# ooowedyn/InkLayer

Hardware: AMD Instinct MI355X
Metric: sketches/sec end-to-end (GroundingDINO+SAM) at 1024x1024 (higher is better)
Workload: dtype f16 (MFMA, f32 accumulate; f32 residual/norm/softmax; split-f16 = fp32-grade operands for patch-embed, neck, mask decoder); 1 GPU; full GroundingDINO Swin-T + SAM ViT-H pipeline, batch=8 per GPU, 1024x1024 synthetic sketches, 16 boxes/sketch, random-init weights; global_batch=8, parallelism=image-parallel x1

## Files before the change

### include/inklayer_hip.h

```cpp
#ifndef INKLAYER_HIP_H
#define INKLAYER_HIP_H

#include <stdint.h>

#ifdef __cplusplus
extern "C" {
#endif

#define INK_ABI_VERSION 10
int ink_abi_version(void);

typedef struct InkGemm {
  const void* A;
  const void* W;
  const float* bias;
  const float* col_scale;
  const float* residual;
  const int32_t* row_map;
  void* C;
  int32_t M, N, K;
  int32_t lda, ldw, ldr, ldc;
  int32_t act;
  int32_t c_f16;
} InkGemm;
// ... 106 lines not shown

int ink_groupnorm_nhwc(const float* x, int32_t B, int32_t T, int32_t C, int32_t G, const float* gamma,
                       const float* beta, float eps, float* stats_ws, float* out,
                       int64_t out_batch_stride, void* stream);

int ink_gather_rows(const float* x, int64_t ldx, int64_t x_batch_rows, const int32_t* idx,
                    int64_t idx_batch_stride, int32_t rows_per_batch, int32_t B, int32_t C,
                    void* out_f16, float* out_f32, void* stream);

int ink_attn_fewkeys(const void* Q, int64_t ldq, const void* K, int64_t ldk, const void* V, int64_t ldv,
                     int32_t B, int32_t n_q, int32_t n_k, int32_t n_heads, int32_t head_dim, float scale,
                     const uint8_t* blocked, const int32_t* q_batch_rows, const float* q_add, int32_t io_f32, void* O,
                     int64_t ldo, void* stream);

int ink_attn_midkeys(const void* Q, int64_t ldq, const void* K, int64_t ldk, const void* V, int64_t ldv, int32_t B,
                     int32_t n_q, int32_t n_k, int32_t n_heads, int32_t head_dim, float scale, const uint8_t* blocked,
                     void* O, int64_t ldo, void* stream);

int ink_biattn_wide_workspace(int32_t B, int32_t S, int32_t T, int64_t* out_floats);
int ink_biattn_wide(const void* QV_f16, const void* KL_f16, int32_t B, int32_t S, int32_t T, int32_t E, float scale,
                    float* ws, void* out_v_f16, void* out_l_f16, void* stream);

int ink_attn_fewq(const void* Q, int64_t ldq, const void* K, int64_t ldk, const void* V, int64_t ldv,
                  int32_t n_batch, int32_t n_q, int32_t n_k, int32_t n_heads, int32_t head_dim, float scale,
                  const int32_t* q_batch_rows, const int32_t* kv_batch_rows, const float* k_add, void* O, int64_t ldo,
                  void* stream);

int ink_biattn_colstats(const float* scores, int32_t B, int32_t S, int32_t HT, float* part_ws, float* stats, void* stream);

int ink_fusion_fold_workspace(int32_t B, int32_t S, int64_t* out_floats);
int ink_fusion_fold(float* v_f32, int32_t B, int32_t S, const float* lnv_g, const float* lnv_b, float eps,
                    const float* text_k_f32, const float* text_vl_f32, int64_t ld_text, int32_t T, const void* Wq_f16,
                    const float* bq, const void* Wvv_f16, const float* bvv, const void* Wo_f16, const float* bo,
                    const float* gamma_v, float scale, float* ws, void* out_l_f16, const float* pos, void* out16_pos,
                    void* out16, void* stream);

int ink_sam_upscale_pack(const void* ws_f16, void* blob_f16, void* stream);
int ink_sam_upscale_tail(const float* u0, int64_t ld_tok, int32_t n, int32_t g, const float* ln_g, const float* ln_b, float eps,
                         const void* blob_f16, const float* b3, const float* hyper, int32_t n_masks, float* low,
                         void* stream);

int ink_proj256_ln_pack(const void* ws_f16, void* blob_f16, void* stream);
int ink_proj256_ln(const float* a_f32, const void* blob_f16, const float* bias, const float* res_f32,
                   const int32_t* res_batch_rows, int32_t rows_per_batch, const float* ln_g, const float* ln_b, float eps,
                   int64_t rows, float* out_f32, void* out_split_f16, void* stream);

int ink_ffn256_pack_bytes(int32_t hid, int32_t with_pre, int64_t* out_bytes);
int ink_ffn256_pack(const void* w1_f16, const float* b1, const void* w2_f16, int32_t hid, const void* wpre_f16, void* blob,
                    void* stream);
int ink_ffn256_fused(const void* x_f16, int64_t ldx, const float* res_f32, const void* blob, const float* b2,
                     const float* ln_g, const float* ln_b, float eps, int32_t M, int32_t hid, const float* pre_bias,
                     const float* pre_ln_g, const float* pre_ln_b, float* out_f32, void* stream);

int ink_topk_rowmax(const float* logits, int32_t B, int32_t S, int32_t T, int32_t K, int32_t* out_idx,
                    float* out_val, void* cand_ws, void* stream);

int ink_sine_embed4(const float* ref, const float* dim_t, int32_t N, void* out_f16, void* stream);

int ink_box_refine(const float* delta, int64_t ldd, const float* ref, int32_t N, int32_t ref_is_logit,
                   float* out, void* stream);

int ink_mask_cleanup_workspace_ints(int32_t n, int32_t H, int32_t W, int32_t k, int64_t* out_ints);
int ink_mask_cleanup(const void* masks_u8, int32_t n, int32_t H, int32_t W, int32_t k, int32_t area_threshold,
                     double aspect_threshold, void* tmp_a_u8, void* tmp_b_u8, int32_t* workspace, void* out_u8,
                     void* stream);

int ink_mask_sketch_iou_counts(const void* masks_u8, const void* sketch_rgb_u8, int32_t n, int32_t H, int32_t W,
                               void* bits_ws_u64, int32_t* counts, void* stream);

int ink_sam_amg_stats(const float* low, int32_t n, const int32_t* index, int32_t m, const int32_t* m_dev, int32_t S,
                      int32_t L, int32_t in_h, int32_t in_w, int32_t crop_h, int32_t crop_w, double thr, double offset,
                      int32_t x0, int32_t y0, int32_t orig_h, int32_t orig_w, int32_t* table, void* planes_u64,
                      float* out_logits, void* stream);

int ink_mask_rle_counts(const void* planes_u64, const int32_t* select, int32_t k, int32_t H, int32_t W,
                        int32_t* n_counts, void* stream);
int ink_mask_rle_write(const void* planes_u64, const int32_t* select, int32_t k, int32_t H, int32_t W,
                       const int32_t* offsets, int32_t* counts, void* stream);

int ink_mask_small_regions_workspace_ints(int32_t k, int32_t H, int32_t W, int64_t* out_ints);
int ink_mask_small_regions(const void* planes_u64, int32_t k, int32_t H, int32_t W, int32_t min_area, int32_t holes,
                           void* tmp_planes_u64, int32_t* workspace, void* out_planes_u64, int32_t* changed, void* stream);

int ink_box_nms(const float* boxes, const float* scores, int32_t n, float iou_threshold, void* workspace_u64,
                int32_t* keep, int32_t* n_keep, void* stream);

int ink_refine_sketch_planes(const void* rgb_u8, int32_t H, int32_t W, void* planes4_u64, int32_t* max_ws, void* stream);

int ink_bitplane_pack(const void* img_u8, int32_t n, int32_t H, int32_t W, int32_t thresh, void* planes_u64, void* stream);

int ink_refine_depth_samples(const void* mask_planes, int32_t n, const float* depth, const int32_t* pts_yx, int32_t P,
                             int32_t H, int32_t W, float* vals, void* inside_u8, void* stream);

int ink_refine_pair_tables(const void* mask_planes, const void* sketch_planes4, int32_t n, int32_t H, int32_t W,
                           const int32_t* rect, void* dil_ws_planes, int32_t* pair, int32_t* per_mask,
                           int32_t* sketch_area, void* stream);

int ink_refine_composite(const void* mask_planes, const int32_t* order, int32_t n_ranks, int32_t H, int32_t W,
                         void* label_u8, int32_t* hist256, void* stream);

int ink_refine_relabel_clean(const void* label_u8, const void* map256_u8, int32_t H, int32_t W, void* out_label_u8,
                             void* stream);

int ink_refine_grow_workspace(int32_t H, int32_t W, int64_t* plane_words, int64_t* cc_ints);
int ink_refine_grow(const void* label_u8, const void* sketch_planes4, int32_t H, int32_t W, void* planes_ws,
                    int32_t* cc_ws, int32_t* flags256, void* out_label_u8, int32_t* bbox256x4, int32_t* unl_yx,
// ... 104 lines not shown
```

### inklayer_amd/_lib.py

```python
from __future__ import annotations

import ctypes as C
import os
from pathlib import Path

_LIB_PATH = Path(__file__).resolve().parent / "lib" / "libinklayer_hip.so"
_lib = None

c_void_p, c_int, c_i64, c_float = C.c_void_p, C.c_int32, C.c_int64, C.c_float


class InkGemm(C.Structure):
    _fields_ = [
        ("A", c_void_p), ("W", c_void_p), ("bias", c_void_p), ("col_scale", c_void_p),
        ("residual", c_void_p), ("row_map", c_void_p), ("C", c_void_p),
        ("M", c_int), ("N", c_int), ("K", c_int),
        ("lda", c_int), ("ldw", c_int), ("ldr", c_int), ("ldc", c_int),
        ("act", c_int), ("c_f16", c_int),
    ]


class InkAttn(C.Structure):
    _fields_ = [
        ("Q", c_void_p), ("K", c_void_p), ("V", c_void_p), ("O", c_void_p),
# ... 20 lines not shown
    "ink_flash_attn": [C.POINTER(InkAttn), c_void_p],
    "ink_swin_attn": [c_void_p, c_void_p, c_void_p, c_i64, c_i64, c_i64, c_void_p, c_i64, c_int, c_int, c_int, c_float,
                      c_void_p, c_void_p, c_int, c_void_p],
    "ink_sam_patchify": [c_void_p, c_int, c_int, c_int, c_int, C.POINTER(c_float), C.POINTER(c_float),
                         c_int, c_int, c_void_p, c_void_p],
    "ink_im2col3x3_f16": [c_void_p, c_int, c_int, c_int, c_int, c_int, c_int, c_void_p, c_void_p],
    "ink_resize_u8": [c_void_p, c_int, c_int, c_int, c_void_p, c_int, c_int, c_void_p, c_void_p, c_int,
                      c_void_p, c_void_p, c_int, c_void_p, c_void_p],
    "ink_sam_pe_encode": [c_void_p, c_void_p, c_int, c_int, c_void_p, c_int, c_void_p, c_void_p],
    "ink_sam_mask_logits": [c_void_p, c_void_p, c_int, c_int, c_int, c_void_p, c_void_p],
    "ink_sam_prompt_tokens": [c_void_p, c_void_p, c_int, c_int, c_void_p, c_void_p, c_int, c_void_p, c_void_p,
                              c_void_p, c_float, c_int, c_void_p, c_void_p],
    "ink_sam_mask_embed": [c_void_p, c_void_p, c_void_p, c_void_p, c_int, c_float, c_int, c_int, c_void_p, c_void_p,
                           c_void_p],
    "ink_sam_postprocess": [c_void_p, c_int, c_int, c_int, c_int, c_int, c_int, c_int, c_float,
                            c_void_p, c_void_p, c_void_p],
    "ink_sam_amg_stats": [c_void_p, c_int, c_void_p, c_int, c_void_p, c_int, c_int, c_int, c_int, c_int, c_int, C.c_double,
                          C.c_double, c_int, c_int, c_int, c_int, c_void_p, c_void_p, c_void_p, c_void_p],
    "ink_mask_rle_counts": [c_void_p, c_void_p, c_int, c_int, c_int, c_void_p, c_void_p],
    "ink_mask_rle_write": [c_void_p, c_void_p, c_int, c_int, c_int, c_void_p, c_void_p, c_void_p],
    "ink_mask_small_regions_workspace_ints": [c_int, c_int, c_int, C.POINTER(c_i64)],
    "ink_mask_small_regions": [c_void_p, c_int, c_int, c_int, c_int, c_int, c_void_p, c_void_p, c_void_p, c_void_p,
                               c_void_p],
    "ink_box_nms": [c_void_p, c_void_p, c_int, c_float, c_void_p, c_void_p, c_void_p, c_void_p],
    "ink_ms_deform_attn_forward": [c_void_p, C.POINTER(c_i64), C.POINTER(c_i64), c_void_p, c_void_p, c_int,
                                   c_int, c_int, c_int, c_int, c_int, c_int, c_int, c_void_p, c_void_p],
    "ink_ms_deform_attn_forward_dev": [c_void_p, c_void_p, c_void_p, c_void_p, c_void_p, c_int, c_int, c_int, c_int,
                                       c_int, c_int, c_int, c_int, c_int, c_void_p, c_void_p],
    "ink_ms_deform_attn_backward_dev": [c_void_p, c_void_p, c_void_p, c_void_p, c_void_p, c_void_p, c_int, c_int, c_int,
                                        c_int, c_int, c_int, c_int, c_int, c_int, c_void_p, c_void_p, c_void_p,
                                        c_void_p],
    "ink_msda_fused": [c_void_p, c_void_p, c_i64, c_void_p, c_int, c_i64, c_i64, C.POINTER(c_int), c_int,
                       c_int, c_int, c_void_p, c_void_p],
    "ink_swin_patchify": [c_void_p, c_int, c_int, C.POINTER(c_float), C.POINTER(c_float), c_void_p, c_void_p],
    "ink_layernorm_merge4": [c_void_p, c_i64, c_void_p, c_void_p, c_float, c_void_p, c_int, c_int, c_void_p,
                             c_void_p],
    "ink_groupnorm_nhwc": [c_void_p, c_int, c_int, c_int, c_int, c_void_p, c_void_p, c_float, c_void_p,
                           c_void_p, c_i64, c_void_p],
    "ink_gather_rows": [c_void_p, c_i64, c_i64, c_void_p, c_i64, c_int, c_int, c_int, c_void_p, c_void_p,
                        c_void_p],
    "ink_biattn_colstats": [c_void_p, c_int, c_int, c_int, c_void_p, c_void_p, c_void_p],
    "ink_fusion_fold_workspace": [c_int, c_int, C.POINTER(c_i64)],
    "ink_relpos_bias64_f16": [c_void_p, c_i64, c_void_p, c_void_p, c_int, c_int, c_int, c_float, c_void_p, c_void_p, c_void_p],
    "ink_proj256_ln_pack": [c_void_p, c_void_p, c_void_p],
    "ink_proj256_ln": [c_void_p, c_void_p, c_void_p, c_void_p, c_void_p, c_int, c_void_p, c_void_p, c_float, c_i64, c_void_p,
                       c_void_p, c_void_p],
    "ink_sam_upscale_pack": [c_void_p, c_void_p, c_void_p],
    "ink_sam_upscale_tail": [c_void_p, c_i64, c_int, c_int, c_void_p, c_void_p, c_float, c_void_p, c_void_p, c_void_p,
                             c_int, c_void_p, c_void_p],
    "ink_ffn256_pack_bytes": [c_int, c_int, C.POINTER(c_i64)],
    "ink_ffn256_pack": [c_void_p, c_void_p, c_void_p, c_int, c_void_p, c_void_p, c_void_p],
    "ink_ffn256_fused": [c_void_p, c_i64, c_void_p, c_void_p, c_void_p, c_void_p, c_void_p, c_float, c_int, c_int,
                         c_void_p, c_void_p, c_void_p, c_void_p, c_void_p],
    "ink_fusion_fold": [c_void_p, c_int, c_int, c_void_p, c_void_p, c_float, c_void_p, c_void_p, c_i64, c_int, c_void_p,
                        c_void_p, c_void_p, c_void_p, c_void_p, c_void_p, c_void_p, c_float, c_void_p, c_void_p, c_void_p,
                        c_void_p, c_void_p, c_void_p],
    "ink_attn_fewkeys": [c_void_p, c_i64, c_void_p, c_i64, c_void_p, c_i64, c_int, c_int, c_int, c_int, c_int,
                         c_float, c_void_p, c_void_p, c_void_p, c_int, c_void_p, c_i64, c_void_p],
    "ink_attn_midkeys": [c_void_p, c_i64, c_void_p, c_i64, c_void_p, c_i64, c_int, c_int, c_int, c_int, c_int,
                         c_float, c_void_p, c_void_p, c_i64, c_void_p],
    "ink_biattn_wide_workspace": [c_int, c_int, c_int, C.POINTER(c_i64)],
    "ink_biattn_wide": [c_void_p, c_void_p, c_int, c_int, c_int, c_int, c_float, c_void_p, c_void_p, c_void_p,
                        c_void_p],
    "ink_attn_fewq": [c_void_p, c_i64, c_void_p, c_i64, c_void_p, c_i64, c_int, c_int, c_int, c_int, c_int,
                      c_float, c_void_p, c_void_p, c_void_p, c_void_p, c_i64, c_void_p],
    "ink_topk_rowmax": [c_void_p, c_int, c_int, c_int, c_int, c_void_p, c_void_p, c_void_p, c_void_p],
    "ink_sine_embed4": [c_void_p, c_void_p, c_int, c_void_p, c_void_p],
    "ink_box_refine": [c_void_p, c_i64, c_void_p, c_int, c_int, c_void_p, c_void_p],
    "ink_mask_cleanup_workspace_ints": [c_int, c_int, c_int, c_int, C.POINTER(c_i64)],
    "ink_mask_cleanup": [c_void_p, c_int, c_int, c_int, c_int, c_int, C.c_double, c_void_p, c_void_p, c_void_p,
                         c_void_p, c_void_p],
    "ink_mask_sketch_iou_counts": [c_void_p, c_void_p, c_int, c_int, c_int, c_void_p, c_void_p, c_void_p],
    "ink_refine_sketch_planes": [c_void_p, c_int, c_int, c_void_p, c_void_p, c_void_p],
    "ink_bitplane_pack": [c_void_p, c_int, c_int, c_int, c_int, c_void_p, c_void_p],
    "ink_refine_depth_samples": [c_void_p, c_int, c_void_p, c_void_p, c_int, c_int, c_int, c_void_p, c_void_p, c_void_p],
    "ink_refine_pair_tables": [c_void_p, c_void_p, c_int, c_int, c_int, c_void_p, c_void_p, c_void_p, c_void_p,
                               c_void_p, c_void_p],
    "ink_refine_composite": [c_void_p, c_void_p, c_int, c_int, c_int, c_void_p, c_void_p, c_void_p],
    "ink_refine_relabel_clean": [c_void_p, c_void_p, c_int, c_int, c_void_p, c_void_p],
    "ink_refine_grow_workspace": [c_int, c_int, C.POINTER(c_i64), C.POINTER(c_i64)],
    "ink_refine_grow": [c_void_p, c_void_p, c_int, c_int, c_void_p, c_void_p, c_void_p, c_void_p, c_void_p, c_void_p,
                        c_int, c_void_p, c_void_p],
    "ink_refine_query_dists": [c_void_p, c_void_p, c_void_p, c_int, c_int, c_int, c_void_p, c_void_p],
    "ink_refine_finalize": [c_void_p, c_void_p, c_int, c_void_p, c_int, c_int, c_void_p, c_void_p, c_void_p, c_void_p],
    "ink_host_sparse_sample": [c_void_p, c_int, c_int, c_void_p, c_int, c_void_p],
    "ink_host_assign_unlabeled": [c_void_p, c_int, c_void_p, c_int, c_void_p, c_void_p, c_void_p, c_int, c_void_p],
    "ink_depth_patchify": [c_void_p, c_int, c_int, c_int, c_int, c_int, c_int, C.POINTER(C.c_double), C.POINTER(C.c_double),
                           c_int, c_void_p, c_void_p],
    "ink_resize_bilinear_ac_nhwc": [c_void_p, c_int, c_int, c_int, c_int, c_int, c_int, c_void_p, c_void_p, c_void_p],
    "ink_conv3x3_f16": [c_void_p, c_int, c_int, c_int, c_int, c_void_p, c_int, c_void_p, c_int, c_int, c_int, c_void_p,
                        c_void_p, c_int, c_void_p],
    "ink_layers_otsu_planes": [c_void_p, c_int, c_int, c_int, c_int, c_void_p, c_void_p, c_void_p, c_void_p],
    "ink_layers_dilate": [c_void_p, c_int, c_int, c_int, c_int, c_int, c_void_p, c_void_p, c_void_p],
    "ink_layers_border_band": [c_void_p, c_int, c_int, c_int, c_int, c_void_p, c_void_p],
    "ink_layers_components_workspace_ints": [c_int, c_int, c_int, C.POINTER(c_i64)],
    "ink_layers_components": [c_void_p, c_int, c_int, c_int, c_int, c_void_p, c_void_p, c_void_p, c_void_p],
    "ink_layers_chamfer_workspace_ints": [c_int, c_int, c_int, C.POINTER(c_i64)],
    "ink_layers_chamfer": [c_void_p, c_void_p, c_int, c_int, c_int, c_int, c_int, c_void_p, c_void_p, c_void_p, c_void_p,
                           c_void_p, c_void_p],
    "ink_layers_mask_tables": [c_void_p, c_int, c_int, c_int, c_void_p, c_void_p, c_void_p],
    "ink_layers_assemble": [c_void_p, c_void_p, c_void_p, c_void_p, c_void_p, c_int, c_int, c_int, c_void_p, c_void_p,
                            c_void_p, c_void_p],
    "ink_layers_composite": [c_void_p, c_void_p, c_int, c_int, c_void_p, c_void_p],
    "ink_layers_gray": [c_void_p, c_int, c_int, c_int, c_void_p, c_void_p],
    "ink_layers_rgba": [c_void_p, c_void_p, c_int, c_int, c_int, c_void_p, c_void_p],
    "ink_inp_contrast": [c_void_p, c_int, c_int, c_float, c_void_p, c_void_p, c_void_p],
# ... 53 lines not shown
```

### inklayer_amd/build.py

```python
from __future__ import annotations

import os
import subprocess
import sys
from concurrent.futures import ThreadPoolExecutor
from pathlib import Path

ROOT = Path(__file__).resolve().parent
CSRC = ROOT / "csrc"
LIBDIR = ROOT / "lib"
OBJDIR = LIBDIR / "obj"
LIB = LIBDIR / "libinklayer_hip.so"
HIPCC = os.environ.get("HIPCC", "/opt/rocm/bin/hipcc")
FLAGS = ["--offload-arch=gfx950", "-O3", "-std=c++17", "-fPIC", "-ffp-contract=off",
         "-mllvm", "-amdgpu-mfma-vgpr-form",

         "-Wall", "-Wno-unused-function", "-Wno-unused-variable"]


def _newest_header() -> float:
    hs = list(CSRC.glob("*.h")) + list((ROOT.parent / "include").glob("*.h"))
    return max(h.stat().st_mtime for h in hs)


NO_SPILL = {"ffn_fused.hip", "proj_ln.hip", "amg.hip", "layers.hip", "inpaint_ops.hip", "visualize.hip", "evaluate.hip",
            "gemm.hip", "attention_swin.hip", "biattn_wide.hip"}


def _check_no_spill(src: Path, remarks: str) -> None:
    name = None
    for line in remarks.splitlines():
        if "Function Name:" in line:
            name = line.split("Function Name:")[1].split("[")[0].strip()
        elif "ScratchSize [bytes/lane]:" in line:
            n = int(line.split("ScratchSize [bytes/lane]:")[1].split("[")[0])
            if n != 0:
                raise RuntimeError(f"{src.name}: kernel {name} spills ({n} bytes of scratch per lane) - the kernels of "
                                   f"this file must stay in registers (see NO_SPILL); reduce register pressure")


def _compile(src: Path, force: bool, hdr_time: float) -> Path:
    obj = OBJDIR / (src.stem + ".o")
    if (not force and obj.exists() and obj.stat().st_mtime > src.stat().st_mtime
            and obj.stat().st_mtime > hdr_time):
        return obj
    guard = src.name in NO_SPILL
    cmd = [HIPCC, *FLAGS, *(["-Rpass-analysis=kernel-resource-usage", "-fno-caret-diagnostics"] if guard else []), "-c", str(src), "-o", str(obj)]
    r = subprocess.run(cmd, capture_output=True, text=True)
    if r.returncode != 0:
        raise RuntimeError(f"hipcc failed for {src.name}:\n{r.stdout}\n{r.stderr}")
    err = r.stderr
    if guard:
        try:
            _check_no_spill(src, err)
        except RuntimeError:
            obj.unlink(missing_ok=True)
            raise
        err = "\n".join(l for l in err.splitlines()
                        if "kernel-resource-usage" not in l and not l.startswith("In file included from"))
    if err.strip():
        sys.stderr.write(err)
    return obj


def build(force: bool = False, verbose: bool = True) -> Path:
    OBJDIR.mkdir(parents=True, exist_ok=True)
    srcs = sorted(CSRC.glob("*.hip"))
    if not srcs:
        raise RuntimeError("no HIP sources found")
    hdr_time = _newest_header()
    with ThreadPoolExecutor(max_workers=min(8, len(srcs))) as ex:
        objs = list(ex.map(lambda s: _compile(s, force, hdr_time), srcs))
    if (force or not LIB.exists()
            or any(o.stat().st_mtime > LIB.stat().st_mtime for o in objs)):
        cmd = [HIPCC, "--offload-arch=gfx950", "-shared", "-fPIC", "-o", str(LIB),
               *map(str, objs)]
        r = subprocess.run(cmd, capture_output=True, text=True)
        if r.returncode != 0:
            raise RuntimeError(f"link failed:\n{r.stdout}\n{r.stderr}")
# ... 8 lines not shown
```

### inklayer_amd/gdino.py

```python
from __future__ import annotations

import math
from dataclasses import dataclass, replace
from typing import Dict, List, Optional, Sequence, Tuple

import numpy as np
import torch

from . import ops
from ._lru import LRU

F16, F32, I32 = torch.float16, torch.float32, torch.int32


@dataclass
class GDinoConfig:
    embed_dim: int = 96
    depths: Tuple[int, ...] = (2, 2, 6, 2)
    num_heads: Tuple[int, ...] = (3, 6, 12, 24)
    window_size: int = 7
    out_indices: Tuple[int, ...] = (1, 2, 3)
    hidden_dim: int = 256
    nheads: int = 8
    enc_layers: int = 6
# ... 287 lines not shown
        return {(k[7:] if k.startswith("module.") else k): v for k, v in sd.items()}
    return sd


class GDinoEngine:
    fuse_ffn = True
    fuse_ffn_pre = True
    fold_fusion = True

    def __init__(self, state_dict: Dict[str, torch.Tensor], cfg: Optional[GDinoConfig] = None,
                 device: str | torch.device = "cuda", encoded_text: Optional[torch.Tensor] = None,
                 token_ids: Sequence[int] = DEFAULT_TOKEN_IDS):
        cfg = cfg or GDinoConfig()
        self.cfg, self.dev = cfg, torch.device(device)
        assert self.dev.type == "cuda", "the InkLayer detector runs on MI355X only"
        check_config(cfg)
        sd, dev = clean_state_dict(state_dict), self.dev
        self.w: Dict[str, torch.Tensor] = {}
        w = self.w

        def h(name, shape=None):
            t = sd[name].detach().to(torch.float32)
            return (t.reshape(shape) if shape is not None else t).to(dev, F16).contiguous()

        def f(name):
            return ops.own_f32(sd[name], dev)

        def lin(dst, src):
            w[dst + ".w"], w[dst + ".b"] = h(src + ".weight"), f(src + ".bias")

        def ln(dst, src):
            w[dst + ".w"], w[dst + ".b"] = f(src + ".weight"), f(src + ".bias")

        def cat_lin(dst, srcs):
            w[dst + ".w"] = torch.cat([h(s + ".weight") for s in srcs]).contiguous()
            w[dst + ".b"] = torch.cat([f(s + ".bias") for s in srcs]).contiguous()

        bb = "backbone.0."
        pw = sd[bb + "patch_embed.proj.weight"].detach().to(torch.float32).cpu().reshape(cfg.embed_dim, 48)
        w["pe.w"] = torch.cat([pw, torch.zeros(cfg.embed_dim, 16)], 1).to(dev, F16).contiguous()
        w["pe.b"] = f(bb + "patch_embed.proj.bias")
        ln("pe.norm", bb + "patch_embed.norm")
        ws = cfg.window_size
        scale = HEAD_DIM ** -0.5
        for i, (dep, nh) in enumerate(zip(cfg.depths, cfg.num_heads)):
            for b in range(dep):
                p, d = f"{bb}layers.{i}.blocks.{b}.", f"s{i}b{b}"
                ln(d + ".norm1", p + "norm1")
                ln(d + ".norm2", p + "norm2")
                lin(d + ".qkv", p + "attn.qkv")
                lin(d + ".proj", p + "attn.proj")
                lin(d + ".fc1", p + "mlp.fc1")
                lin(d + ".fc2", p + "mlp.fc2")
                tab = sd[p + "attn.relative_position_bias_table"].detach().to(torch.float32).cpu()
                if ws == 7:
                    w[d + ".bias"] = swin_dense_bias(tab, ws, nh, scale).to(dev).contiguous()
                else:
                    w[d + ".table"] = swin_bias_table(tab, ws, nh).to(dev).contiguous()
            if i < len(cfg.depths) - 1:
                ln(f"s{i}.merge.norm", f"{bb}layers.{i}.downsample.norm")
                w[f"s{i}.merge.w"] = h(f"{bb}layers.{i}.downsample.reduction.weight")
            if i in cfg.out_indices:
                ln(f"s{i}.outnorm", f"{bb}norm{i}")
        for l in range(cfg.num_feature_levels):
            cw = sd[f"input_proj.{l}.0.weight"].detach().to(torch.float32)
            if cw.shape[-1] == 1:
                w[f"ip{l}.w"] = cw.reshape(cw.shape[0], cw.shape[1]).to(dev, F16).contiguous()
            else:
                w[f"ip{l}.w"] = cw.permute(0, 2, 3, 1).reshape(cw.shape[0], -1).to(dev, F16).contiguous()
            w[f"ip{l}.b"] = f(f"input_proj.{l}.0.bias")
            ln(f"ip{l}.gn", f"input_proj.{l}.1")
        t = "transformer."
        self.level_embed_cpu = sd[t + "level_embed"].detach().to(torch.float32).cpu()

        def msda(dst, src):
            cat_lin(dst + ".proj", [src + "sampling_offsets", src + "attention_weights"])
            lin(dst + ".value", src + "value_proj")
            lin(dst + ".out", src + "output_proj")

        def mha(dst, src):
            W, b = sd[src + "in_proj_weight"].detach().to(torch.float32), sd[src + "in_proj_bias"].detach().to(torch.float32)
            D = W.shape[1]
            w[dst + ".qk.w"], w[dst + ".qk.b"] = W[:2 * D].to(dev, F16).contiguous(), b[:2 * D].to(dev).contiguous()
            w[dst + ".q.w"], w[dst + ".q.b"] = W[:D].to(dev, F16).contiguous(), b[:D].to(dev).contiguous()
            w[dst + ".kv.w"], w[dst + ".kv.b"] = W[D:].to(dev, F16).contiguous(), b[D:].to(dev).contiguous()
            w[dst + ".v.w"], w[dst + ".v.b"] = W[2 * D:].to(dev, F16).contiguous(), b[2 * D:].to(dev).contiguous()
            lin(dst + ".out", src + "out_proj")

        for i in range(cfg.enc_layers):
            p, d = f"{t}encoder.layers.{i}.", f"e{i}"
            msda(d + ".msda", p + "self_attn.")
            ln(d + ".norm1", p + "norm1"); lin(d + ".lin1", p + "linear1"); lin(d + ".lin2", p + "linear2"); ln(d + ".norm2", p + "norm2")
            if w[d + ".lin1.w"].shape[1] == 256 and w[d + ".lin1.w"].shape[0] % 64 == 0 and w[d + ".lin1.w"].shape[0] <= 2048:
                w[d + ".ffn.blob"] = ops.ffn256_pack(w[d + ".lin1.w"], w[d + ".lin1.b"], w[d + ".lin2.w"])
                w[d + ".ffn.blob_pre"] = ops.ffn256_pack(w[d + ".lin1.w"], w[d + ".lin1.b"], w[d + ".lin2.w"],
                                                         w[d + ".msda.out.w"])
            p = f"{t}encoder.text_layers.{i}."
            mha(d + ".txt", p + "self_attn.")
            lin(d + ".txt.lin1", p + "linear1"); lin(d + ".txt.lin2", p + "linear2")
            ln(d + ".txt.norm1", p + "norm1"); ln(d + ".txt.norm2", p + "norm2")
            p = f"{t}encoder.fusion_layers.{i}."
            ln(d + ".fu.lnv", p + "layer_norm_v"); ln(d + ".fu.lnl", p + "layer_norm_l")
            cat_lin(d + ".fu.qv", [p + "attn.v_proj", p + "attn.values_v_proj"])
            cat_lin(d + ".fu.kl", [p + "attn.l_proj", p + "attn.values_l_proj"])
            lin(d + ".fu.outv", p + "attn.out_v_proj"); lin(d + ".fu.outl", p + "attn.out_l_proj")
            w[d + ".fu.gv"], w[d + ".fu.gl"] = f(p + "gamma_v"), f(p + "gamma_l")
# ... 41 lines not shown
        self._graphs.clear()
        self._seen.clear()
        self.T = T
        self.token_ids = tuple(int(t) for t in token_ids)
        self._text_attn = ops.attn_fewkeys if T <= 16 else ops.attn_midkeys
        self.text0 = encoded_text.detach().to(self.dev, F32).contiguous()
        self._captions.put(self.token_ids, encoded_text.detach().to("cpu", F32))
        self.Tc, self.logit_bias = -(-T // 4) * 4, None
        if self.Tc != T:
            self.logit_bias = torch.zeros(self.Tc, dtype=F32)
            self.logit_bias[T:] = float("-inf")
            self.logit_bias = self.logit_bias.to(self.dev)
        sm, pid = text_masks_and_position_ids(token_ids)
        self.text_blocked = (~sm).to(torch.uint8).to(self.dev).contiguous()
        dim_t = torch.arange(256, dtype=torch.float32)
        dim_t = 10000.0 ** (2 * torch.div(dim_t, 2, rounding_mode="floor") / 256)
        self.pos_text = _interleaved_sincos(pid.float()[:, None] * (2 * math.pi) / dim_t).to(self.dev).contiguous()

    caption_cache_size = 8
    tokenizer = None

    def set_caption(self, token_ids: Sequence[int], sd: Optional[Dict[str, torch.Tensor]] = None,
                    encoded_text: Optional[torch.Tensor] = None) -> None:
        ids = tuple(int(t) for t in token_ids)[:self.cfg.max_text_len]
        if sd is not None:
            sd = clean_state_dict(sd)
            self.text_weights = {k: v for k, v in sd.items() if k.startswith(("bert.", "feat_map."))}
            self._captions.clear()
        if encoded_text is None:
            encoded_text = self._captions.get(ids)
        if encoded_text is None:
            if not self.text_weights:
                raise ValueError("set_caption needs encoded_text [T, 256] or a state dict with the checkpoint's bert.* "
                                 "and feat_map.* tensors")
            from .text_branch import encode_caption_from_checkpoint
            encoded_text = encode_caption_from_checkpoint(self.text_weights, ids)
        self.set_text(encoded_text[:len(ids)], ids)

    def predict(self, images_u8: Sequence[torch.Tensor], box_threshold: float, text_threshold: float,
                remove_combined: bool = False):
        logits, boxes = self.forward(images_u8)
        both = torch.cat([logits, boxes], dim=-1).cpu()
        T, res = self.T, []
        for b in range(both.shape[0]):
            prob = both[b, :, :T].contiguous().sigmoid()
            keep = prob.max(dim=1)[0] > box_threshold
            kept = prob[keep]
            phrases = phrases_from_probs(kept, self.token_ids, text_threshold, remove_combined, self.tokenizer)
            res.append((both[b, keep, T:], kept.max(dim=1)[0] if len(kept) else kept.new_zeros(0), phrases))
        return res

    graph_max_batch = 1
    graph_cache_size = 4
    plan_cache_size = 8

    def _forward_graphed(self, images_u8: Sequence[torch.Tensor], h: int, w_: int):
        B = len(images_u8)
        key = (h, w_, B)
        g = self._graphs.get(key)
        if g is None:
            self._seen[key] = self._seen.get(key, 0) + 1
            if len(self._seen) > 4096:
                self._seen.clear()
            if self._seen[key] < 2:
                return self._forward_eager(images_u8)
            static_in = [torch.empty_like(im) for im in images_u8]
            for dst, src in zip(static_in, images_u8):
                dst.copy_(src)
            side = torch.cuda.Stream(device=self.dev)
            side.wait_stream(torch.cuda.current_stream(self.dev))
            with torch.cuda.stream(side):
                for _ in range(2):
                    self._forward_eager(static_in)
            torch.cuda.current_stream(self.dev).wait_stream(side)
            graph = torch.cuda.CUDAGraph()
            with torch.cuda.graph(graph):
                out = self._forward_eager(static_in)
            g = (graph, static_in, out, self.plan(h, w_, B))
            self._graphs.put(key, g)
        graph, static_in, out = g[:3]
        for dst, src in zip(static_in, images_u8):
            dst.copy_(src)
        graph.replay()
        return out[0].clone(), out[1].clone()

    def plan(self, h: int, w: int, B: int) -> _Plan:
        return self._plans.get_or_make((h, w, B), lambda: _Plan(self, h, w, B))

    def _mlp3(self, prefix: str, x16: torch.Tensor) -> torch.Tensor:
        w = self.w
        a = ops.gemm(x16, w[prefix + "0.w"], w[prefix + "0.b"], act="relu", out_dtype=F16)
        a = ops.gemm(a, w[prefix + "1.w"], w[prefix + "1.b"], act="relu", out_dtype=F16)
        return ops.gemm(a, w[prefix + "2.w"], w[prefix + "2.b"])

    def _swin_block(self, x: torch.Tensor, i: int, b: int, pl: _Plan) -> None:
        cfg, w = self.cfg, self.w
        C, nh, nW = cfg.embed_dim * 2 ** i, cfg.num_heads[i], pl.nW[i]
        d = f"s{i}b{b}"
        shifted = b % 2 == 1
        wm = pl.win_map[i][1 if shifted else 0]
        y = ops.layernorm_rows(x, w[d + ".norm1.w"], w[d + ".norm1.b"], 1e-5, gather=wm)
        qkv = ops.gemm(y, w[d + ".qkv.w"], w[d + ".qkv.b"], out_dtype=F16)
        ws, scale = cfg.window_size, HEAD_DIM ** -0.5
        if ws == 7:
            o = ops.flash_attn(qkv[:, :C], qkv[:, C:2 * C], qkv[:, 2 * C:], n_batch=pl.B * nW, n_heads=nh,
                               head_dim=HEAD_DIM, scale=scale, n_q=ws * ws, n_k=ws * ws, dense_bias=w[d + ".bias"],
                               dense_mask=pl.shift_mask[i] if shifted else None)
        else:
            o = ops.swin_attn(qkv[:, :C], qkv[:, C:2 * C], qkv[:, 2 * C:], n_windows=pl.B * nW, n_heads=nh, ws=ws,
                              scale=scale, bias_table=w[d + ".table"], region=pl.region[i] if shifted else None, nW=nW)
        ops.gemm(o, w[d + ".proj.w"], w[d + ".proj.b"], residual=x, row_map=wm, out=x)
        y = ops.layernorm_rows(x, w[d + ".norm2.w"], w[d + ".norm2.b"], 1e-5)
        hmid = ops.gemm(y, w[d + ".fc1.w"], w[d + ".fc1.b"], act="gelu", out_dtype=F16)
        ops.gemm(hmid, w[d + ".fc2.w"], w[d + ".fc2.b"], residual=x, out=x)

    def backbone(self, images_u8: Sequence[torch.Tensor], pl: _Plan) -> Dict[int, Tuple[torch.Tensor, torch.Tensor]]:
        cfg, w, dev = self.cfg, self.w, self.dev
        B = len(images_u8)
        H0, W0 = pl.stage_hw[0]
        T0 = H0 * W0
        patches = torch.empty((B * T0, 64), device=dev, dtype=F16)
        for b, img in enumerate(images_u8):
            ops.swin_patchify(img, cfg.pixel_mean, cfg.pixel_std, patches[b * T0:(b + 1) * T0])
        x = ops.gemm(patches, w["pe.w"], w["pe.b"])
        x = ops.layernorm_rows(x, w["pe.norm.w"], w["pe.norm.b"], 1e-5, out_dtype=F32)
        outs = {}
        for i, dep in enumerate(cfg.depths):
            for b in range(dep):
                self._swin_block(x, i, b, pl)
            if i in cfg.out_indices:
                o32 = torch.empty_like(x)
                o16 = torch.empty(x.shape, device=dev, dtype=F16)
                ops.layernorm_rows(x, w[f"s{i}.outnorm.w"], w[f"s{i}.outnorm.b"], 1e-5, out=o32, out2=o16)
                outs[i] = (o32, o16)
            if i < len(cfg.depths) - 1:
                m = ops.layernorm_merge4(x, w[f"s{i}.merge.norm.w"], w[f"s{i}.merge.norm.b"], 1e-5, pl.merge_map[i])
                x = ops.gemm(m, w[f"s{i}.merge.w"])
        return outs

    def neck(self, feats, pl: _Plan, B: int) -> torch.Tensor:
        cfg, w, dev = self.cfg, self.w, self.dev
        S = pl.S
        src = torch.empty((B * S, 256), device=dev, dtype=F32)
        nfeat = len(cfg.out_indices)
        for l in range(cfg.num_feature_levels):
            hh, ww = pl.shapes[l]
            Tl = hh * ww
            if l < nfeat:
                a16 = feats[cfg.out_indices[l]][1]
            else:
                f32_last = feats[cfg.out_indices[-1]][0]
                T3 = pl.shapes[nfeat - 1][0] * pl.shapes[nfeat - 1][1]
                col = ops.gather_rows(f32_last, pl.lvl4_map, B, Tl * 9, x_batch_rows=T3, idx_batch_stride=0)
                a16 = col.view(B * Tl, -1)
            y = ops.gemm(a16, w[f"ip{l}.w"], w[f"ip{l}.b"])
            ops.groupnorm_nhwc(y, B, Tl, 32, w[f"ip{l}.gn.w"], w[f"ip{l}.gn.b"], 1e-5,
                               src[pl.level_start[l]:], S * 256)
        return src

    def encoder(self, src: torch.Tensor, pl: _Plan, B: int):
        S = pl.S
        text = self.text0.repeat(B, 1)
        s16 = torch.empty((B * S, 256), device=self.dev, dtype=F16)
        s16p = torch.empty((B * S, 256), device=self.dev, dtype=F16)
# ... 186 lines not shown
```

### inklayer_amd/ops.py

```python
from __future__ import annotations

import ctypes as C
from typing import Optional, Sequence, Tuple

import torch

from . import _lib
from ._lib import InkAttn, InkGemm, check

ACT = {None: 0, "none": 0, "gelu": 1, "relu": 2}
F16, F32 = torch.float16, torch.float32


_GEMM_TRACE = None


def set_gemm_trace(lst) -> None:
    global _GEMM_TRACE
    _GEMM_TRACE = lst


_ATTN_TRACE = None


# ... 781 lines not shown

def sam_upscale_tail(u0: torch.Tensor, n: int, g: int, ln_g: torch.Tensor, ln_b: torch.Tensor, eps: float,
                     blob: torch.Tensor, b3: torch.Tensor, hyper: torch.Tensor) -> torch.Tensor:
    if u0.shape[1] == 64:
        assert u0.is_contiguous() and u0.shape[0] == n * g * g * 4
        u0 = u0.view(n * g * g, 256)
    assert u0.dtype == F32 and u0.stride(1) == 1 and tuple(u0.shape) == (n * g * g, 256) and u0.stride(0) % 4 == 0
    assert blob.dtype == F16 and blob.numel() == 4 * 12 * 64 * 8 and b3.dtype == F32 and b3.numel() == 128
    assert hyper.dtype == F32 and hyper.is_contiguous() and hyper.dim() == 3 and hyper.shape[0] == n and hyper.shape[2] == 32
    assert ln_g.dtype == F32 and ln_b.dtype == F32 and ln_g.numel() == 64 and ln_b.numel() == 64
    M = hyper.shape[1]
    low = torch.empty((n, M, 4 * g, 4 * g), device=u0.device, dtype=F32)
    check(_lib.lib().ink_sam_upscale_tail(_p(u0), u0.stride(0), n, g, _p(ln_g), _p(ln_b), eps, _p(blob), _p(b3), _p(hyper), M,
                                          _p(low), _stream()), "ink_sam_upscale_tail")
    return low


def ffn256_pack(w1: torch.Tensor, b1: torch.Tensor, w2: torch.Tensor, w_pre: Optional[torch.Tensor] = None) -> torch.Tensor:
    hid = int(w1.shape[0])
    assert w1.dtype == F16 and w2.dtype == F16 and w1.is_contiguous() and w2.is_contiguous()
    assert tuple(w1.shape) == (hid, 256) and tuple(w2.shape) == (256, hid)
    assert b1.dtype == F32 and b1.is_contiguous() and b1.numel() == hid
    assert w_pre is None or (w_pre.dtype == F16 and w_pre.is_contiguous() and tuple(w_pre.shape) == (256, 256))
    need = C.c_int64(0)
    check(_lib.lib().ink_ffn256_pack_bytes(hid, int(w_pre is not None), C.byref(need)), "ink_ffn256_pack_bytes")
    blob = torch.empty(need.value // 2, device=w1.device, dtype=F16)
    check(_lib.lib().ink_ffn256_pack(w1.data_ptr(), b1.data_ptr(), w2.data_ptr(), hid, _p(w_pre), blob.data_ptr(), _stream()),
          "ink_ffn256_pack")
    return blob


def ffn256_fused(x16: torch.Tensor, res: torch.Tensor, blob: torch.Tensor, hid: int, b2: torch.Tensor,
                 ln_g: torch.Tensor, ln_b: torch.Tensor, eps: float, out: Optional[torch.Tensor] = None,
                 pre: Optional[Tuple[torch.Tensor, torch.Tensor, torch.Tensor]] = None) -> torch.Tensor:
    M = int(x16.shape[0])
    assert x16.dtype == F16 and x16.stride(1) == 1 and x16.shape[1] == 256
    assert res.dtype == F32 and res.is_contiguous() and tuple(res.shape) == (M, 256)
    need = C.c_int64(0)
    check(_lib.lib().ink_ffn256_pack_bytes(hid, int(pre is not None), C.byref(need)), "ink_ffn256_pack_bytes")
    assert blob.dtype == F16 and blob.numel() * 2 == need.value and b2.dtype == F32
    assert b2.numel() == 256 and ln_g.numel() == 256 and ln_b.numel() == 256 and ln_g.dtype == F32 and ln_b.dtype == F32
    if pre is not None:
        assert all(t.dtype == F32 and t.is_contiguous() and t.numel() == 256 for t in pre)
    if out is None:
        out = torch.empty_like(res)
    assert out.dtype == F32 and out.is_contiguous() and tuple(out.shape) == (M, 256)
    pb, pg, pe = pre if pre is not None else (None, None, None)
    check(_lib.lib().ink_ffn256_fused(x16.data_ptr(), x16.stride(0), res.data_ptr(), blob.data_ptr(), b2.data_ptr(),
                                      ln_g.data_ptr(), ln_b.data_ptr(), eps, M, hid, _p(pb), _p(pg), _p(pe), out.data_ptr(),
                                      _stream()), "ink_ffn256_fused")
    return out


def attn_fewkeys(q: torch.Tensor, k: torch.Tensor, v: torch.Tensor, *, B: int, n_heads: int, head_dim: int,
                 scale: float, blocked: Optional[torch.Tensor] = None, n_q: Optional[int] = None,
                 q_batch_rows: Optional[torch.Tensor] = None, q_add: Optional[torch.Tensor] = None) -> torch.Tensor:
    io = q.dtype
    for t in (q, k, v):
        assert t.dtype == io and io in (F16, F32) and t.dim() == 2 and t.stride(1) == 1
        assert t.data_ptr() % 16 == 0
    if n_q is None:
        n_q = q.shape[0] // B
    n_k = k.shape[0] // B
    out = torch.empty((B * n_q, n_heads * head_dim), device=q.device, dtype=io)
    if blocked is not None:
        assert blocked.dtype == torch.uint8 and blocked.is_contiguous() and blocked.shape == (n_q, n_k)
    if q_batch_rows is not None:
        assert q_batch_rows.dtype == torch.int32 and q_batch_rows.numel() == B and q_batch_rows.is_cuda
    if q_add is not None:
        assert q_add.dtype == F32 and q_add.is_contiguous() and tuple(q_add.shape) == (n_q, n_heads * head_dim)
    check(_lib.lib().ink_attn_fewkeys(q.data_ptr(), q.stride(0), k.data_ptr(), k.stride(0), v.data_ptr(),
                                      v.stride(0), B, n_q, n_k, n_heads, head_dim, scale, _p(blocked),
                                      _p(q_batch_rows), _p(q_add), int(io == F32), out.data_ptr(), out.stride(0), _stream()),
          "ink_attn_fewkeys")
    return out


def attn_midkeys(q: torch.Tensor, k: torch.Tensor, v: torch.Tensor, *, B: int, n_heads: int, head_dim: int,
                 scale: float, blocked: Optional[torch.Tensor] = None) -> torch.Tensor:
    for t in (q, k, v):
        assert t.dtype == F16 and t.dim() == 2 and t.stride(1) == 1
        assert t.data_ptr() % 16 == 0
    n_q, n_k = q.shape[0] // B, k.shape[0] // B
    out = torch.empty((B * n_q, n_heads * head_dim), device=q.device, dtype=F16)
    if blocked is not None:
        assert blocked.dtype == torch.uint8 and blocked.is_contiguous() and blocked.shape == (n_q, n_k)
    check(_lib.lib().ink_attn_midkeys(q.data_ptr(), q.stride(0), k.data_ptr(), k.stride(0), v.data_ptr(), v.stride(0),
                                      B, n_q, n_k, n_heads, head_dim, scale, _p(blocked), out.data_ptr(),
                                      out.stride(0), _stream()), "ink_attn_midkeys")
    return out


def attn_fewq(q: torch.Tensor, k: torch.Tensor, v: torch.Tensor, *, n_batch: int, n_heads: int, head_dim: int,
              scale: float, n_q: int, n_k: int, q_batch_rows: Optional[torch.Tensor] = None,
              kv_batch_rows: Optional[torch.Tensor] = None, k_add: Optional[torch.Tensor] = None) -> torch.Tensor:
    for t in (q, k, v):
        assert t.dtype == F32 and t.dim() == 2 and t.stride(1) == 1
        assert t.data_ptr() % 16 == 0
    for rows in (q_batch_rows, kv_batch_rows):
        assert rows is None or (rows.dtype == torch.int32 and rows.numel() == n_batch and rows.is_cuda)
    out = torch.empty((n_batch * n_q, n_heads * head_dim), device=q.device, dtype=F32)
    if k_add is not None:
        assert k_add.dtype == F32 and k_add.is_contiguous() and tuple(k_add.shape) == (n_k, n_heads * head_dim)
    check(_lib.lib().ink_attn_fewq(q.data_ptr(), q.stride(0), k.data_ptr(), k.stride(0), v.data_ptr(), v.stride(0),
                                   n_batch, n_q, n_k, n_heads, head_dim, scale, _p(q_batch_rows),
                                   _p(kv_batch_rows), _p(k_add), out.data_ptr(), out.stride(0), _stream()),
# ... 452 lines not shown
```

Measured before the change: 118.7 sketches/s.

## Fuse Swin MLP LayerNorm, fc1+GELU, fc2 and residual into one kernel

```diff
diff --git a/include/inklayer_hip.h b/include/inklayer_hip.h
--- a/include/inklayer_hip.h
+++ b/include/inklayer_hip.h
@@ -182,6 +182,12 @@
                      const float* ln_g, const float* ln_b, float eps, int32_t M, int32_t hid, const float* pre_bias,
                      const float* pre_ln_g, const float* pre_ln_b, float* out_f32, void* stream);
 
+int ink_swin_mlp_pack_bytes(int32_t C, int32_t hid, int64_t* out_bytes);
+int ink_swin_mlp_pack(const void* w1_f16, const float* b1, const void* w2_f16, int32_t C, int32_t hid, void* blob,
+                      void* stream);
+int ink_swin_mlp_fused(float* x_f32, int64_t ld, int32_t M, int32_t C, const void* blob, int32_t hid, const float* b2,
+                       const float* ln_g, const float* ln_b, float eps, void* stream);
+
 int ink_topk_rowmax(const float* logits, int32_t B, int32_t S, int32_t T, int32_t K, int32_t* out_idx,
                     float* out_val, void* cand_ws, void* stream);
 
diff --git a/inklayer_amd/_lib.py b/inklayer_amd/_lib.py
--- a/inklayer_amd/_lib.py
+++ b/inklayer_amd/_lib.py
@@ -96,6 +96,10 @@
     "ink_ffn256_pack": [c_void_p, c_void_p, c_void_p, c_int, c_void_p, c_void_p, c_void_p],
     "ink_ffn256_fused": [c_void_p, c_i64, c_void_p, c_void_p, c_void_p, c_void_p, c_void_p, c_float, c_int, c_int,
                          c_void_p, c_void_p, c_void_p, c_void_p, c_void_p],
+    "ink_swin_mlp_pack_bytes": [c_int, c_int, C.POINTER(c_i64)],
+    "ink_swin_mlp_pack": [c_void_p, c_void_p, c_void_p, c_int, c_int, c_void_p, c_void_p],
+    "ink_swin_mlp_fused": [c_void_p, c_i64, c_int, c_int, c_void_p, c_int, c_void_p, c_void_p, c_void_p, c_float,
+                           c_void_p],
     "ink_fusion_fold": [c_void_p, c_int, c_int, c_void_p, c_void_p, c_float, c_void_p, c_void_p, c_i64, c_int, c_void_p,
                         c_void_p, c_void_p, c_void_p, c_void_p, c_void_p, c_void_p, c_float, c_void_p, c_void_p, c_void_p,
                         c_void_p, c_void_p, c_void_p],
diff --git a/inklayer_amd/build.py b/inklayer_amd/build.py
--- a/inklayer_amd/build.py
+++ b/inklayer_amd/build.py
@@ -24,7 +24,7 @@
 
 
 NO_SPILL = {"ffn_fused.hip", "proj_ln.hip", "amg.hip", "layers.hip", "inpaint_ops.hip", "visualize.hip", "evaluate.hip",
-            "gemm.hip", "attention_swin.hip", "biattn_wide.hip"}
+            "gemm.hip", "attention_swin.hip", "biattn_wide.hip", "swin_mlp.hip"}
 
 
 def _check_no_spill(src: Path, remarks: str) -> None:
diff --git a/inklayer_amd/csrc/swin_mlp.hip b/inklayer_amd/csrc/swin_mlp.hip
--- /dev/null
+++ b/inklayer_amd/csrc/swin_mlp.hip
@@ -0,0 +1,265 @@
+#include "mfma_util.h"
+#include "../../include/inklayer_hip.h"
+
+namespace {
+
+constexpr int HC = 64, BM = 128;
+constexpr int BLK = 1024;
+constexpr int DEPTH = 6;
+
+template <int C>
+struct Geo {
+  static constexpr int KA = C / 16 + 1;
+  static constexpr int W1_BLKS = (HC / 32) * KA;
+  static constexpr int W2_BLKS = (C / 32) * (HC / 16);
+  static constexpr int NBLK = W1_BLKS + W2_BLKS;
+  static constexpr int CHUNK = NBLK * BLK;
+  static constexpr int NSLOT = (NBLK + 3) / 4;
+  static constexpr int ROWB = C * 4 + 16;
+  static constexpr int PR = C / 4;
+  static constexpr int NP = BM * PR / 256;
+  static constexpr int PAR = 2 * CHUNK;
+  static constexpr int LDS_BYTES = 2 * CHUNK + 3 * C * 4;
+  static_assert(C % 32 == 0 && NBLK % 4 == 2, "one DMA piece per four MFMAs covers the chunk");
+  static_assert(BM * ROWB <= 2 * CHUNK, "row staging fits the weight buffers");
+  static_assert(LDS_BYTES <= 160 * 1024, "LDS budget");
+};
+
+__host__ __device__ constexpr bool width_ok(int C) { return C == 96 || C == 192; }
+__host__ __device__ constexpr int64_t chunk_bytes(int C) { return (int64_t)(2 * (C / 16 + 1) + (C / 32) * (HC / 16)) * BLK; }
+
+__host__ __device__ constexpr int hid_perm(int p) { return (p & 7) < 4 ? 4 * (p >> 3) + (p & 7) : 8 + 4 * (p >> 3) + (p & 7) - 4; }
+
+__global__ __launch_bounds__(256) void swin_mlp_pack_kernel(const f16* __restrict__ W1, const float* __restrict__ b1,
+                                                            const f16* __restrict__ W2, int C, int HID,
+                                                            f16* __restrict__ blob) {
+  const int64_t idx = (int64_t)blockIdx.x * 256 + threadIdx.x;
+  const int KA = C / 16 + 1, W1_BLKS = (HC / 32) * KA, NBLK = W1_BLKS + (C / 32) * (HC / 16);
+  const int64_t total = (int64_t)(HID / HC) * NBLK * 64;
+  if (idx >= total) return;
+  const int lane = (int)(idx & 63);
+  const int q = (int)((idx >> 6) % NBLK);
+  const int c = (int)((idx >> 6) / NBLK);
+  const int l = lane & 31, hh = lane >> 5;
+  f16x8 v = {0, 0, 0, 0, 0, 0, 0, 0};
+  if (q < W1_BLKS) {
+    const int jt = q / KA, s = q % KA;
+    const int j = c * HC + 32 * jt + l;
+    if (s < C / 16) {
+      const f16* src = W1 + (int64_t)j * C + 16 * s;
+#pragma unroll
+      for (int e = 0; e < 8; ++e) v[e] = src[hid_perm(8 * hh + e)];
+    } else if (hh == 0) {
+      const f16 hi = (f16)b1[j];
+      v[0] = hi;
+      v[1] = (f16)(b1[j] - (float)hi);
+    }
+  } else {
+    const int nt = (q - W1_BLKS) / (HC / 16), s = (q - W1_BLKS) % (HC / 16);
+    const f16* src = W2 + (int64_t)(32 * nt + l) * HID + c * HC + 16 * s;
+#pragma unroll
+    for (int e = 0; e < 8; ++e) v[e] = src[hid_perm(8 * hh + e)];
+  }
+  *(f16x8*)(blob + idx * 8) = v;
+}
+
+template <int C>
+__global__ __launch_bounds__(256, C <= 96 ? 2 : 1) void swin_mlp_fused_kernel(float* x, int64_t ld, const f16* __restrict__ blob,
+                                                             const float* __restrict__ b2, const float* __restrict__ ln_g,
+                                                             const float* __restrict__ ln_b, float eps, int M, int HID) {
+  using G = Geo<C>;
+  constexpr int KA = G::KA, W1_BLKS = G::W1_BLKS, NBLK = G::NBLK, CHUNK = G::CHUNK, NSLOT = G::NSLOT, ROWB = G::ROWB;
+  constexpr int PR = G::PR, NP = G::NP;
+  extern __shared__ __attribute__((aligned(16))) char smem[];
+  const int tid = threadIdx.x, lane = tid & 63;
+  const int wave = __builtin_amdgcn_readfirstlane(tid >> 6);
+  const int l = lane & 31, hh = lane >> 5;
+  const int ntiles = (M + BM - 1) / BM;
+  const int t0 = xcd_remap(blockIdx.x, ntiles) * BM;
+  const int m0 = t0 + wave * 32;
+  const int nchunk = HID / HC;
+
+  {
+    f32x4 t[NP];
+#pragma unroll
+    for (int k = 0; k < NP; ++k) {
+      const int p = tid + 256 * k, r = p / PR, c4 = p % PR;
+      t[k] = *(const f32x4*)(x + (int64_t)min(t0 + r, M - 1) * ld + c4 * 4);
+    }
+    float* sP = (float*)(smem + G::PAR);
+    for (int i = tid; i < C; i += 256) {
+      sP[i] = ln_g[i];
+      sP[C + i] = ln_b[i];
+      sP[2 * C + i] = b2[i];
+    }
+#pragma unroll
+    for (int k = 0; k < NP; ++k) {
+      const int p = tid + 256 * k, r = p / PR, c4 = p % PR;
+      *(f32x4*)(smem + r * ROWB + c4 * 16) = t[k];
+    }
+  }
+  __syncthreads();
+
+  f32x16 y[C / 32];
+  {
+    const char* rp = smem + (wave * 32 + l) * ROWB + 16 * hh;
+#pragma unroll
+    for (int nt = 0; nt < C / 32; ++nt)
+#pragma unroll
+      for (int g = 0; g < 4; ++g) {
+        const f32x4 r4 = *(const f32x4*)(rp + (32 * nt + 8 * g) * 4);
+#pragma unroll
+        for (int e = 0; e < 4; ++e) y[nt][4 * g + e] = r4[e];
+      }
+  }
+
+  f16x8 xf[KA];
+  const uint32_t par0 = lds_addr(smem) + G::PAR + 16 * hh;
+  {
+    float sum = 0.f;
+#pragma unroll
+    for (int nt = 0; nt < C / 32; ++nt)
+#pragma unroll
+      for (int r = 0; r < 16; ++r) sum += y[nt][r];
+    sum += __shfl_xor(sum, 32, 64);
+    const float mean = sum * (1.0f / C);
+    float sq = 0.f;
+#pragma unroll
+    for (int nt = 0; nt < C / 32; ++nt)
+#pragma unroll
+      for (int r = 0; r < 16; ++r) {
+        const float d = y[nt][r] - mean;
+        sq += d * d;
+      }
+    sq += __shfl_xor(sq, 32, 64);
+    const float rstd = 1.0f / sqrtf(sq * (1.0f / C) + eps);
+    static_for<0, C / 16>([&](auto ii) {
+      constexpr int s = decltype(ii)::value, nt = s / 2, g = 2 * (s % 2);
+      constexpr int o0 = (32 * nt + 8 * g) * 4;
+      f32x4 g0 = lds_f4<o0>(par0), g1 = lds_f4<o0 + 32>(par0), b0 = lds_f4<C * 4 + o0>(par0), b1v = lds_f4<C * 4 + o0 + 32>(par0);
+      wait_f4(g0, g1, b0, b1v);
+#pragma unroll
+      for (int e = 0; e < 4; ++e) {
+        xf[s][e] = (f16)((y[nt][4 * g + e] - mean) * rstd * g0[e] + b0[e]);
+        xf[s][4 + e] = (f16)((y[nt][4 * g + 4 + e] - mean) * rstd * g1[e] + b1v[e]);
+      }
+    });
+    xf[C / 16] = (f16x8){0, 0, 0, 0, 0, 0, 0, 0};
+    if (hh == 0) xf[C / 16][0] = xf[C / 16][1] = (f16)1.0f;
+    static_for<0, C / 32>([&](auto ii) {
+      constexpr int nt = decltype(ii)::value;
+      constexpr int ob = 2 * (C * 4) + (32 * nt) * 4;
+      f32x4 c0 = lds_f4<ob>(par0), c1 = lds_f4<ob + 32>(par0), c2 = lds_f4<ob + 64>(par0), c3 = lds_f4<ob + 96>(par0);
+      wait_f4(c0, c1, c2, c3);
+#pragma unroll
+      for (int e = 0; e < 4; ++e) {
+        y[nt][e] += c0[e];
+        y[nt][4 + e] += c1[e];
+        y[nt][8 + e] += c2[e];
+        y[nt][12 + e] += c3[e];
+      }
+    });
+  }
+  __syncthreads();
+  asm volatile("s_waitcnt vmcnt(0)" ::: "memory");
+
+  auto stage = [&](int buf, int c, int k) {
+    const int q = min(4 * k + wave, NBLK - 1);
+    __builtin_amdgcn_global_load_lds((gptr_t)((const char*)blob + (int64_t)c * CHUNK + q * BLK + lane * 16),
+                                     (lptr_t)(smem + buf * CHUNK + q * BLK), 16, 0, 0);
+  };
+#pragma unroll
+  for (int k = 0; k < NSLOT; ++k) stage(0, 0, k);
+
+  const uint32_t lds0 = lds_addr(smem) + lane * 16;
+  const f32x16 zero = {0.f, 0.f, 0.f, 0.f, 0.f, 0.f, 0.f, 0.f, 0.f, 0.f, 0.f, 0.f, 0.f, 0.f, 0.f, 0.f};
+  for (int c = 0; c < nchunk; ++c) {
+    asm volatile("s_waitcnt vmcnt(0)" ::: "memory");
+    __builtin_amdgcn_s_barrier();
+    asm volatile("" ::: "memory");
+    const int cn = min(c + 1, nchunk - 1);
+    const uint32_t wa = lds0 + (c & 1) * CHUNK;
+    f16x8 fr[DEPTH + 1];
+
+    auto read = [&](auto ii) {
+      constexpr int i = decltype(ii)::value;
+      if constexpr (i < W1_BLKS) fr[i % (DEPTH + 1)] = lds_frag<i * BLK>(wa);
+      else fr[i % (DEPTH + 1)] = lds_frag<(W1_BLKS + ((i - W1_BLKS) % (C / 32)) * (HC / 16) + (i - W1_BLKS) / (C / 32)) * BLK>(wa);
+    };
+    static_for<0, DEPTH>(read);
+    f32x16 h[HC / 32];
+    f16x8 hf[HC / 16];
+    static_for<0, NBLK>([&](auto ii) {
+      constexpr int i = decltype(ii)::value;
+      if constexpr (i + DEPTH < NBLK) read(ic<i + DEPTH>{});
+      wait_frag<(NBLK - 1 - i < DEPTH ? NBLK - 1 - i : DEPTH)>(fr[i % (DEPTH + 1)]);
+      if constexpr (i < W1_BLKS) {
+        constexpr int jt = i / KA, s = i % KA;
+        h[jt] = mfma32(fr[i % (DEPTH + 1)], xf[s], s == 0 ? zero : h[jt]);
+      } else {
+        constexpr int s = (i - W1_BLKS) / (C / 32), nt = (i - W1_BLKS) % (C / 32);
+        if constexpr (nt == 0) {
+#pragma unroll
+          for (int e = 0; e < 8; ++e) hf[s][e] = (f16)gelu_erf(h[s >> 1][8 * (s & 1) + e]);
+        }
+        y[nt] = mfma32(fr[i % (DEPTH + 1)], hf[s], y[nt]);
+      }
+      if constexpr (i % 4 == 1) stage((c + 1) & 1, cn, i / 4);
+    });
+  }
+
+  asm volatile("s_waitcnt vmcnt(0)" ::: "memory");
+  __syncthreads();
+  char* ot = smem + wave * 32 * ROWB;
+#pragma unroll
+  for (int nt = 0; nt < C / 32; ++nt)
+#pragma unroll
+    for (int g = 0; g < 4; ++g) {
+      f32x4 v;
+#pragma unroll
+      for (int e = 0; e < 4; ++e) v[e] = y[nt][4 * g + e];
+      *(f32x4*)(ot + l * ROWB + (32 * nt + 8 * g + 4 * hh) * 4) = v;
+    }
+#pragma unroll 4
+  for (int k = 0; k < 32 * PR / 64; ++k) {
+    const int p = lane + 64 * k, r = p / PR, c4 = p % PR;
+    const int m = m0 + r;
+    if (m < M) *(f32x4*)(x + (int64_t)m * ld + c4 * 4) = *(const f32x4*)(ot + r * ROWB + c4 * 16);
+  }
+}
+
+template <int C>
+void launch(float* x, int64_t ld, const void* blob, const float* b2, const float* ln_g, const float* ln_b, float eps,
+            int M, int hid, hipStream_t stream) {
+  ink_dyn_lds<swin_mlp_fused_kernel<C>>(Geo<C>::LDS_BYTES);
+  hipLaunchKernelGGL(swin_mlp_fused_kernel<C>, dim3((M + BM - 1) / BM), dim3(256), Geo<C>::LDS_BYTES, stream, x, ld,
+                     (const f16*)blob, b2, ln_g, ln_b, eps, M, hid);
+}
+
+}
+
+extern "C" int ink_swin_mlp_pack_bytes(int32_t C, int32_t hid, int64_t* out_bytes) {
+  INK_CHECK_ARG(out_bytes && width_ok(C) && hid > 0 && hid % HC == 0);
+  *out_bytes = (int64_t)(hid / HC) * chunk_bytes(C);
+  return INK_OK;
+}
+
+extern "C" int ink_swin_mlp_pack(const void* w1_f16, const float* b1, const void* w2_f16, int32_t C, int32_t hid, void* blob,
+                                 void* stream) {
+  INK_CHECK_ARG(w1_f16 && b1 && w2_f16 && blob && width_ok(C) && hid > 0 && hid % HC == 0);
+  INK_CHECK_ARG(ink_aligned<16>(w1_f16, w2_f16, blob) && ink_aligned<4>(b1));
+  const int64_t pieces = (int64_t)(hid / HC) * (chunk_bytes(C) / 16);
+  hipLaunchKernelGGL(swin_mlp_pack_kernel, dim3((unsigned)((pieces + 255) / 256)), dim3(256), 0, (hipStream_t)stream,
+                     (const f16*)w1_f16, b1, (const f16*)w2_f16, C, hid, (f16*)blob);
+  return ink_launch_status();
+}
+
+extern "C" int ink_swin_mlp_fused(float* x_f32, int64_t ld, int32_t M, int32_t C, const void* blob, int32_t hid,
+                                  const float* b2, const float* ln_g, const float* ln_b, float eps, void* stream) {
+  INK_CHECK_ARG(x_f32 && blob && b2 && ln_g && ln_b);
+  INK_CHECK_ARG(M > 0 && width_ok(C) && hid > 0 && hid % HC == 0 && ld >= C && ld % 4 == 0);
+  INK_CHECK_ARG(ink_aligned<16>(x_f32, blob, b2, ln_g, ln_b));
+  if (C == 96) launch<96>(x_f32, ld, blob, b2, ln_g, ln_b, eps, M, hid, (hipStream_t)stream);
+  else launch<192>(x_f32, ld, blob, b2, ln_g, ln_b, eps, M, hid, (hipStream_t)stream);
+  return ink_launch_status();
+}
diff --git a/inklayer_amd/gdino.py b/inklayer_amd/gdino.py
--- a/inklayer_amd/gdino.py
+++ b/inklayer_amd/gdino.py
@@ -363,6 +363,8 @@
                 lin(d + ".proj", p + "attn.proj")
                 lin(d + ".fc1", p + "mlp.fc1")
                 lin(d + ".fc2", p + "mlp.fc2")
+                if ops.swin_mlp_supported(cfg.embed_dim * 2 ** i):
+                    w[d + ".mlp.blob"] = ops.swin_mlp_pack(w[d + ".fc1.w"], w[d + ".fc1.b"], w[d + ".fc2.w"])
                 tab = sd[p + "attn.relative_position_bias_table"].detach().to(torch.float32).cpu()
                 if ws == 7:
                     w[d + ".bias"] = swin_dense_bias(tab, ws, nh, scale).to(dev).contiguous()
@@ -510,6 +512,7 @@
 
     graph_max_batch = 1
     graph_cache_size = 4
+    swin_mlp_fused = True
     plan_cache_size = 8
 
     def _forward_graphed(self, images_u8: Sequence[torch.Tensor], h: int, w_: int):
@@ -568,6 +571,10 @@
             o = ops.swin_attn(qkv[:, :C], qkv[:, C:2 * C], qkv[:, 2 * C:], n_windows=pl.B * nW, n_heads=nh, ws=ws,
                               scale=scale, bias_table=w[d + ".table"], region=pl.region[i] if shifted else None, nW=nW)
         ops.gemm(o, w[d + ".proj.w"], w[d + ".proj.b"], residual=x, row_map=wm, out=x)
+        if self.swin_mlp_fused and d + ".mlp.blob" in w:
+            ops.swin_mlp_fused(x, w[d + ".mlp.blob"], int(w[d + ".fc1.b"].numel()), w[d + ".fc2.b"], w[d + ".norm2.w"],
+                               w[d + ".norm2.b"], 1e-5)
+            return
         y = ops.layernorm_rows(x, w[d + ".norm2.w"], w[d + ".norm2.b"], 1e-5)
         hmid = ops.gemm(y, w[d + ".fc1.w"], w[d + ".fc1.b"], act="gelu", out_dtype=F16)
         ops.gemm(hmid, w[d + ".fc2.w"], w[d + ".fc2.b"], residual=x, out=x)
diff --git a/inklayer_amd/ops.py b/inklayer_amd/ops.py
--- a/inklayer_amd/ops.py
+++ b/inklayer_amd/ops.py
@@ -857,6 +857,38 @@
     return out
 
 
+def swin_mlp_supported(width: int) -> bool:
+    need = C.c_int64(0)
+    return _lib.lib().ink_swin_mlp_pack_bytes(int(width), 64, C.byref(need)) == 0
+
+
+def swin_mlp_pack(w1: torch.Tensor, b1: torch.Tensor, w2: torch.Tensor) -> torch.Tensor:
+    hid, Cw = int(w1.shape[0]), int(w1.shape[1])
+    assert w1.dtype == F16 and w2.dtype == F16 and w1.is_contiguous() and w2.is_contiguous()
+    assert tuple(w2.shape) == (Cw, hid)
+    assert b1.dtype == F32 and b1.is_contiguous() and b1.numel() == hid
+    need = C.c_int64(0)
+    check(_lib.lib().ink_swin_mlp_pack_bytes(Cw, hid, C.byref(need)), "ink_swin_mlp_pack_bytes")
+    blob = torch.empty(need.value // 2, device=w1.device, dtype=F16)
+    check(_lib.lib().ink_swin_mlp_pack(w1.data_ptr(), b1.data_ptr(), w2.data_ptr(), Cw, hid, blob.data_ptr(), _stream()),
+          "ink_swin_mlp_pack")
+    return blob
+
+
+def swin_mlp_fused(x: torch.Tensor, blob: torch.Tensor, hid: int, b2: torch.Tensor, ln_w: torch.Tensor,
+                   ln_b: torch.Tensor, eps: float) -> torch.Tensor:
+    M, Cw = int(x.shape[0]), int(x.shape[1])
+    assert x.dtype == F32 and x.dim() == 2 and x.stride(1) == 1
+    need = C.c_int64(0)
+    check(_lib.lib().ink_swin_mlp_pack_bytes(Cw, hid, C.byref(need)), "ink_swin_mlp_pack_bytes")
+    assert blob.dtype == F16 and blob.numel() * 2 == need.value
+    for t in (b2, ln_w, ln_b):
+        assert t.dtype == F32 and t.is_contiguous() and t.numel() == Cw
+    check(_lib.lib().ink_swin_mlp_fused(x.data_ptr(), x.stride(0), M, Cw, blob.data_ptr(), hid, b2.data_ptr(),
+                                        ln_w.data_ptr(), ln_b.data_ptr(), eps, _stream()), "ink_swin_mlp_fused")
+    return x
+
+
 def attn_fewkeys(q: torch.Tensor, k: torch.Tensor, v: torch.Tensor, *, B: int, n_heads: int, head_dim: int,
                  scale: float, blocked: Optional[torch.Tensor] = None, n_q: Optional[int] = None,
                  q_batch_rows: Optional[torch.Tensor] = None, q_add: Optional[torch.Tensor] = None) -> torch.Tensor:
```

Result: no change. 119.4 sketches/s, median of 6 (+0.6%).
